# facebookresearch/goliath

Hardware: AMD Instinct MI355X
Metric: relit views/sec (fwd+bwd) at 2048x1334, 250k Gaussians (higher is better)
Workload: dtype f32; 1 GPU; rgca_config2_envrelight; gaussians=250000, views_per_gpu=8, micro_batches=2, world_size=1, dist_backend=none, rccl_world_size=0, parallelism=view-parallel x1, launch=hip_graph_replay

## Files before the change

goliath_amd/_lib.py:

```python
import ctypes
import os

import torch

_HERE = os.path.dirname(os.path.abspath(__file__))
LIB_PATH = os.environ.get("GOLIATH_HIP_LIB") or os.path.join(_HERE, "lib", "libgoliath_hip.so")

_lib = None

_SYMBOLS = [
    "gol_version", "gol_last_error", "gol_sg_eval_fwd", "gol_sg_eval_bwd", "gol_project_fwd",
    "gol_project_bwd", "gol_project_bwd_records", "gol_bin_sort", "gol_splat_pack", "gol_render_layout", "gol_render_fwd", "gol_render_bwd", "gol_rasterize_fwd", "gol_rasterize_bwd", "gol_rasterize_nd_fwd", "gol_rasterize_nd_bwd", "gol_raster_plan", "gol_raster_count_pairs", "gol_shade_fwd",
    "gol_shade_bwd", "gol_shade_project_fwd", "gol_shade_project_bwd", "gol_render_layout_projected", "gol_render_fwd_projected",
    "gol_render_bwd_projected", "gol_selftest_wave_sum4", "gol_selftest_wave_sum8", "gol_raydirs_fwd", "gol_mvp_aabb", "gol_mvp_march_fwd",
    "gol_mvp_march_bwd", "gol_mvp_march_warp_fwd", "gol_mvp_march_warp_bwd", "gol_envmap_pack", "gol_uvlight_phong_fwd", "gol_uvlight_phong_bwd",
    "gol_uvlight_ggx_fwd", "gol_uvlight_ggx_bwd", "gol_l1_blocks", "gol_l1_fwd", "gol_l1_bwd",
    "gol_tail_conv_fwd", "gol_tail_conv_bwd", "gol_tail_conv_bwd_scratch_floats", "gol_ssim_blocks", "gol_ssim_fwd", "gol_ssim_bwd",
    "gol_shadow_pcf", "gol_imgtail_partial_floats", "gol_imgtail_fwd", "gol_imgtail_bwd", "gol_mvp_shadow_march", "gol_mesh_raster_workspace_bytes", "gol_mesh_raster",
    "gol_mesh_render_fwd", "gol_mesh_render_bwd", "gol_mesh_render_edge_bwd",
    "gol_vert_normals_fwd", "gol_vert_normals_bwd", "gol_values_to_uv_fwd", "gol_values_to_uv_bwd", "gol_uvgeom_fwd",
    "gol_uvgeom_bwd", "gol_lbs_skeleton_fwd", "gol_lbs_skeleton_bwd", "gol_lbs_skin_fwd", "gol_lbs_skin_bwd",
    "gol_optim_chunk_elems", "gol_optim_grad_stats", "gol_optim_finalize", "gol_optim_adam_step",
    "gol_regloss_chunk_elems", "gol_regloss_fwd", "gol_regloss_bwd", "gol_backlit_fwd", "gol_backlit_bwd",
    "gol_imgloss_chunk_elems", "gol_imgloss_fwd", "gol_imgloss_finalize", "gol_imgloss_bwd", "gol_depth_disc_mask",
    "gol_mask_erode", "gol_envbg_blur_taps", "gol_envbg_scratch_floats", "gol_envbg_image", "gol_envbg_compose",
    "gol_sh_norm_constants", "gol_sh_basis_fwd", "gol_light_sh_fwd", "gol_envspin_scratch_floats", "gol_envspin_frame",
    "gol_mvp_template_fwd", "gol_mvp_template_bwd", "gol_mvp_primtransf_fwd", "gol_mvp_primtransf_bwd",
    "gol_envprefilter_scratch_floats", "gol_envprefilter_sg",
    "gol_trunk_conv_fwd", "gol_trunk_conv_bwd_scratch_floats", "gol_trunk_conv_bwd",
    "gol_enc_conv_fwd", "gol_enc_conv_bwd_scratch_floats", "gol_enc_conv_bwd",
    "gol_mesh_raster_flat", "gol_uv_face_index_workspace_bytes", "gol_uv_face_index", "gol_uv_topology", "gol_nearest_valid", "gol_impaint_gather",
    "gol_face_visibility", "gol_view_texture", "gol_texmean_finalize",
    "gol_uvframes_bwd_scratch_floats", "gol_uvframes_fwd", "gol_uvframes_bwd",
    "gol_upconv_fwd", "gol_upconv_bwd_scratch_floats", "gol_upconv_bwd",
    "gol_upcat_conv_fwd", "gol_upcat_conv_bwd_scratch_floats", "gol_upcat_conv_bwd",
    "gol_uvtex_partial_floats", "gol_uvtex_fwd", "gol_uvtex_bwd", "gol_pack_rgba_fwd", "gol_pack_rgba_bwd",
    "gol_normal_rgba",
    "gol_olat_features_fwd", "gol_olat_combine_fwd", "gol_olat_combine_bwd",
    "gol_mvp_tail_fwd", "gol_mvp_tail_bwd_scratch_floats", "gol_mvp_tail_bwd",
    "gol_conv3_fwd", "gol_conv3_bwd_x",
    "gol_mbconv_front_tiles", "gol_mbconv_front_fwd", "gol_mbconv_front_bwd_x",
]


class GoliathHipError(RuntimeError):
    pass


def load():
    global _lib
    if _lib is None:
        if not os.path.exists(LIB_PATH):
            raise GoliathHipError(
                f"{LIB_PATH} not found: the HIP extension is not built. Run "
                "`python -m goliath_amd.build` (or __graft_entry__.build()). There is no CPU fallback."
            )
        lib = ctypes.CDLL(LIB_PATH)
        lib.gol_version.restype = ctypes.c_char_p
        lib.gol_last_error.restype = ctypes.c_char_p
        for name in _SYMBOLS:
            getattr(lib, name)
        _lib = lib
    return _lib


def exported_symbols():
    return list(_SYMBOLS)
# ... 72 lines not shown
```

goliath_amd/csrc/abi.hip:

```cpp
#include <cstdarg>
#include <cstdio>

#include "gol_common.h"

static thread_local char g_err[512] = "";

void gol_set_error(const char* fmt, ...) {
  va_list ap;
  va_start(ap, fmt);
  vsnprintf(g_err, sizeof(g_err), fmt, ap);
  va_end(ap);
}

extern "C" const char* gol_version(void) { return "goliath_hip 0.1.0 gfx950"; }
extern "C" const char* gol_last_error(void) { return g_err; }

__global__ void selftest_wave_sum4_kernel(const float* __restrict__ in, float* __restrict__ out) {
  const int l = threadIdx.x;
  const float r = gol_wave_sum4(in[l], in[64 + l], in[128 + l], in[192 + l]);
  out[l] = r;
  out[64 + l] = gol_wave_sum_to_lane63(in[l]);
}
extern "C" int gol_selftest_wave_sum4(const float* in256, float* out128, void* stream) {
  selftest_wave_sum4_kernel<<<1, 64, 0, (hipStream_t)stream>>>(in256, out128);
  GOL_CHECK_LAUNCH();
  return GOL_OK;
}

__global__ void selftest_wave_sum8_kernel(const float* __restrict__ in, float* __restrict__ out) {
  const int l = threadIdx.x;
  out[l] = gol_wave_sum8(in[l], in[64 + l], in[128 + l], in[192 + l], in[256 + l], in[320 + l], in[384 + l], in[448 + l]);
}
extern "C" int gol_selftest_wave_sum8(const float* in512, float* out64, void* stream) {
  selftest_wave_sum8_kernel<<<1, 64, 0, (hipStream_t)stream>>>(in512, out64);
  GOL_CHECK_LAUNCH();
  return GOL_OK;
}
```

goliath_amd/csrc/gol_common.h:

```cpp
#pragma once
#include <hip/hip_runtime.h>
#include <type_traits>
#include <stdint.h>

#include "../../include/goliath_hip.h"

#define GOL_BLUR 0.3f
#define GOL_FOV_CLAMP 1.3f
#define GOL_EIG_FLOOR 0.1f
#define GOL_RADIUS_SIGMAS 3.0f
#define GOL_Z_EPS 1e-6f
#define GOL_ALPHA_CAP_FWD 0.999f
#define GOL_ALPHA_CAP_BWD 0.99f
#define GOL_ALPHA_FLOOR (1.f / 255.f)
#define GOL_T_STOP 1e-4f
#define GOL_COMP_EPS 1e-6f

#define GOL_WAVE 64

void gol_set_error(const char* fmt, ...);

#define GOL_REQUIRE(cond, msg)                                         \
  do {                                                                 \
    if (!(cond)) {                                                     \
// ... 23 lines not shown
__device__ __forceinline__ float gol_add_row_shr8(float v) {
  float r;
  asm("s_nop 1\n\tv_add_f32_dpp %0, %1, %1 row_shr:8 row_mask:0xf bank_mask:0xf bound_ctrl:1" : "=v"(r) : "v"(v));
  return r;
}
__device__ __forceinline__ float gol_add_row_bcast15(float v) {
  asm("s_nop 1\n\tv_add_f32_dpp %0, %0, %0 row_bcast:15 row_mask:0xa bank_mask:0xf" : "+v"(v));
  return v;
}
__device__ __forceinline__ float gol_add_row_bcast31(float v) {
  asm("s_nop 1\n\tv_add_f32_dpp %0, %0, %0 row_bcast:31 row_mask:0xc bank_mask:0xf" : "+v"(v));
  return v;
}

__device__ __forceinline__ float gol_row_sum_to_lane15(float v) {
  v += gol_dpp_mov0<0x111>(v);
  v += gol_dpp_mov0<0x112>(v);
  v += gol_dpp_mov0<0x114>(v);
  return gol_add_row_shr8(v);
}

__device__ __forceinline__ float gol_swap32_sum(float x, float y) {
  const auto r = __builtin_amdgcn_permlane32_swap(__builtin_bit_cast(unsigned, x), __builtin_bit_cast(unsigned, y),
                                                  false, false);
  const unsigned r0 = r[0], r1 = r[1];
  return __uint_as_float(r0) + __uint_as_float(r1);
}
__device__ __forceinline__ float gol_swap16_sum(float x, float y) {
  const auto r = __builtin_amdgcn_permlane16_swap(__builtin_bit_cast(unsigned, x), __builtin_bit_cast(unsigned, y),
                                                  false, false);
  const unsigned r0 = r[0], r1 = r[1];
  return __uint_as_float(r0) + __uint_as_float(r1);
}
__device__ __forceinline__ float gol_wave_sum4(float a, float b, float c, float d) {
  const float ac = gol_swap32_sum(a, c);
  const float bd = gol_swap32_sum(b, d);
  const float q = gol_swap16_sum(ac, bd);
  return gol_row_sum_to_lane15(q);
}

__device__ __forceinline__ float gol_wave_sum8(float a0, float a1, float a2, float a3, float a4, float a5, float a6,
                                               float a7) {
  const float p02 = gol_swap32_sum(a0, a2), p13 = gol_swap32_sum(a1, a3);
  const float q02 = gol_swap32_sum(a4, a6), q13 = gol_swap32_sum(a5, a7);
  float p = gol_swap16_sum(p02, p13);
  const float q = gol_swap16_sum(q02, q13);
  p += gol_dpp_mov0<0x128>(p);
  asm("s_nop 1\n\tv_add_f32_dpp %0, %1, %1 row_ror:8 row_mask:0xf bank_mask:0xc" : "+v"(p) : "v"(q));
  p += gol_dpp_mov0<0x111>(p);
  p += gol_dpp_mov0<0x112>(p);
  float r;
  asm("s_nop 1\n\tv_add_f32_dpp %0, %1, %1 row_shr:4 row_mask:0xf bank_mask:0xf bound_ctrl:1" : "=v"(r) : "v"(p));
  return r;
}

template <typename T>
__device__ __forceinline__ T* gol_at(T* base, unsigned byte_off) {
  return reinterpret_cast<T*>(reinterpret_cast<char*>(const_cast<typename std::remove_const<T>::type*>(base)) + byte_off);
}

template <typename T>
__device__ __forceinline__ T* gol_uniform(T* q) {
  const uint64_t v = reinterpret_cast<uint64_t>(q);
  const uint32_t lo = __builtin_amdgcn_readfirstlane((uint32_t)v), hi = __builtin_amdgcn_readfirstlane((uint32_t)(v >> 32));
  return reinterpret_cast<T*>(((uint64_t)hi << 32) | lo);
}

__device__ __forceinline__ unsigned long long gol_ballot(bool p) { return __builtin_amdgcn_ballot_w64(p); }

__device__ __forceinline__ float gol_wave_sum_to_lane63(float v) {
  v += gol_dpp_mov0<0x111>(v);
  v += gol_dpp_mov0<0x112>(v);
  v += gol_dpp_mov0<0x114>(v);
  v = gol_add_row_shr8(v);
  v = gol_add_row_bcast15(v);
  return gol_add_row_bcast31(v);
}

template <int CTRL, int ROW_MASK>
__device__ __forceinline__ double gol_dpp_add0(double v) {
  const int lo = __builtin_amdgcn_update_dpp(0, __double2loint(v), CTRL, ROW_MASK, 0xf, false);
  const int hi = __builtin_amdgcn_update_dpp(0, __double2hiint(v), CTRL, ROW_MASK, 0xf, false);
  return v + __hiloint2double(hi, lo);
}
__device__ __forceinline__ double gol_wave_sum_to_lane63(double v) {
  v = gol_dpp_add0<0x111, 0xf>(v);
  v = gol_dpp_add0<0x112, 0xf>(v);
  v = gol_dpp_add0<0x114, 0xf>(v);
  v = gol_dpp_add0<0x118, 0xf>(v);
  v = gol_dpp_add0<0x142, 0xa>(v);
  return gol_dpp_add0<0x143, 0xc>(v);
}

__device__ __forceinline__ float gol_readlane63(float v) {
  return __builtin_bit_cast(float, __builtin_amdgcn_readlane(__builtin_bit_cast(int, v), 63));
}

__device__ __forceinline__ float gol_alpha_tau(float op) {
  _Pragma("clang fp contract(on)")
  const float k = 255.f * op;
  return (k >= 1.f) ? __logf(k) * 1.001f + 1e-3f : -1.f;
}
__device__ __forceinline__ float gol_min_sigma_rect(float gx, float gy, float a, float b, float c, float ia, float ic,
                                                    float x0, float x1, float y0, float y1) {
  if (gx >= x0 && gx <= x1 && gy >= y0 && gy <= y1) return 0.f;
  float m = 3.0e38f;
// ... 38 lines not shown
```

goliath_amd/csrc/gol_raster.h:

```cpp
#pragma once
#include <type_traits>

#include "gol_common.h"

namespace {

constexpr int kBatch = 256;
constexpr float kUnA = GOL_UN_A, kUnB = GOL_UN_B;
__device__ __forceinline__ float3 true_conic(float a, float b, float c) { return make_float3(a * kUnA, b * kUnB, c * kUnA); }
#ifdef GOL_EXACT_MATH
__device__ __forceinline__ float exact_sigma(float a, float b, float c, float dx, float dy) {
#pragma clang fp contract(off)
  const float t1 = (a * dx) * dx, t2 = (c * dy) * dy, t3 = (b * dx) * dy;
  const float h = 0.5f * (t1 + t2);
  return h + t3;
}
__device__ __forceinline__ float exact_exp_neg(float s) { return (float)exp(-(double)s); }
__device__ __forceinline__ float exact_next_T(float T, float alpha) {
#pragma clang fp contract(off)
  const float om = 1.f - alpha;
  return T * om;
}
#endif

// ... 94 lines not shown
template <int PPL> using ivec = typename Pix<PPL>::iv;

template <int PPL>
__device__ __forceinline__ void visit_falloff(float ca, float cb, float cc, float dx, const fvec<PPL>& dy, fvec<PPL>& sigma,
                                              fvec<PPL>& e) {
#ifndef GOL_EXACT_MATH
  sigma = (ca * dx * dx + cc * dy * dy) + (cb * dx) * dy;
#pragma unroll
  for (int q = 0; q < PPL; ++q) e[q] = __builtin_amdgcn_exp2f(-sigma[q]);
#else
#pragma unroll
  for (int q = 0; q < PPL; ++q) { sigma[q] = exact_sigma(ca, cb, cc, dx, dy[q]); e[q] = exact_exp_neg(sigma[q]); }
#endif
}

template <int PPL>
__device__ __forceinline__ unsigned long long fwd_step(const fvec<PPL>& sigma, fvec<PPL> alpha, const fvec<PPL>& live,
                                                       const fvec<PPL>& T_cur, fvec<PPL>& vis, fvec<PPL>& next_T,
                                                       bool (&take)[PPL], unsigned long long (&stop)[PPL]) {
  alpha *= live;
  vis = alpha * T_cur;
#ifndef GOL_EXACT_MATH
  next_T = T_cur - vis;
#else
#pragma unroll
  for (int q = 0; q < PPL; ++q) next_T[q] = exact_next_T(T_cur[q], alpha[q]);
#endif
  unsigned long long any_stop = 0ull;
#pragma unroll
  for (int q = 0; q < PPL; ++q) {
    const unsigned long long mc = gol_ballot(!(sigma[q] < 0.f)) & gol_ballot(!(alpha[q] < GOL_ALPHA_FLOOR));
    const unsigned long long ms = gol_ballot(next_T[q] <= GOL_T_STOP);
    take[q] = __builtin_amdgcn_inverse_ballot_w64(mc & ~ms);
    stop[q] = mc & ms;
    any_stop |= stop[q];
  }
  return any_stop;
}

template <int PPL>
__device__ __forceinline__ void fwd_take(const bool (&take)[PPL], const fvec<PPL>& next_T, fvec<PPL>& vis, fvec<PPL>& T_cur) {
#pragma unroll
  for (int q = 0; q < PPL; ++q) vis[q] = take[q] ? vis[q] : 0.f;
#ifndef GOL_EXACT_MATH
  T_cur -= vis;
#else
#pragma unroll
  for (int q = 0; q < PPL; ++q) T_cur[q] = take[q] ? next_T[q] : T_cur[q];
#endif
}

template <int PPL>
__device__ __forceinline__ unsigned long long bwd_taken(float opacity, const fvec<PPL>& e, const fvec<PPL>& sigma, int li,
                                                        const ivec<PPL>& bin_final, fvec<PPL>& alpha,
                                                        unsigned long long (&mv)[PPL]) {
  alpha = opacity * e;
  unsigned long long many = 0ull;
#pragma unroll
  for (int q = 0; q < PPL; ++q) {
    alpha[q] = fminf(GOL_ALPHA_CAP_BWD, alpha[q]);
    mv[q] = gol_ballot(li <= bin_final[q]) & gol_ballot(!(sigma[q] < 0.f)) & gol_ballot(!(alpha[q] < GOL_ALPHA_FLOOR));
    many |= mv[q];
  }
  return many;
}

template <int PPL>
__device__ __forceinline__ void bwd_recur(const unsigned long long (&mv)[PPL], fvec<PPL>& alpha, fvec<PPL>& T_cur,
                                          bool (&v)[PPL], fvec<PPL>& ra, fvec<PPL>& fac) {
#pragma unroll
  for (int q = 0; q < PPL; ++q) {
    v[q] = __builtin_amdgcn_inverse_ballot_w64(mv[q]);
    alpha[q] = v[q] ? alpha[q] : 0.f;
  }
  const fvec<PPL> one_m = 1.f - alpha;
#pragma unroll
  for (int q = 0; q < PPL; ++q) ra[q] = __builtin_amdgcn_rcpf(one_m[q]);
  const fvec<PPL> T_new = T_cur * ra;
  fac = alpha * T_new;
  T_cur = T_new;
}

template <int PPL>
__device__ __forceinline__ void bwd_moments(const fvec<PPL>& e, const fvec<PPL>& w, const fvec<PPL>& T_cur,
                                            const fvec<PPL>& alpha, const bool (&v)[PPL], const fvec<PPL>& dy,
                                            fvec<PPL>& R, fvec<PPL>& gop, fvec<PPL>& gy, fvec<PPL>& gyy) {
  const fvec<PPL> d = w - R;
  const fvec<PPL> v_alpha = T_cur * d;
  R += alpha * d;
  gop = e * v_alpha;
#pragma unroll
  for (int q = 0; q < PPL; ++q) gop[q] = v[q] ? gop[q] : 0.f;
  gy = gop * dy;
  gyy = gy * dy;
}
template <int PPL>
__device__ __forceinline__ float lane_sum(const fvec<PPL>& x) {
  float s = x[0];
#pragma unroll
  for (int q = 1; q < PPL; ++q) s += x[q];
  return s;
}

template <int PPL>
__device__ __forceinline__ int wave_last_entry(const ivec<PPL>& bin_final) {
  int wmax = bin_final[0];
#pragma unroll
  for (int q = 1; q < PPL; ++q) wmax = max(wmax, bin_final[q]);
#pragma unroll
  for (int off = 32; off > 0; off >>= 1) wmax = max(wmax, __shfl_xor(wmax, off, 64));
  return __builtin_amdgcn_readfirstlane(wmax);
}

inline int64_t raster_grid(int B, int img_h, int img_w) {
  return (int64_t)B * 8 * (((img_h + 15) / 16 + 7) / 8) * ((img_w + 15) / 16);
}

#define GOL_RASTER_CHECK_DIMS(bytes_per_pixel, too_large_msg)                                                           \
  do {                                                                                                                  \
    GOL_REQUIRE(B >= 0 && N >= 0, "negative size");                                                                     \
    GOL_REQUIRE(block == 16, "only block_width == 16 is implemented (the reference's value, render_gsplat.py:28)");     \
    GOL_REQUIRE(img_h > 0 && img_w > 0, "empty image");                                                                 \
    GOL_REQUIRE(raster_grid(B, img_h, img_w) < (1ll << 31), "too many tiles");                                          \
    GOL_REQUIRE((uint64_t)img_h * (uint64_t)img_w * (uint64_t)(bytes_per_pixel) < (1ull << 32), too_large_msg);         \
  } while (0)

template <typename F>
inline void with_ppl(int ppl, F&& fn) {
  if (ppl == 2) fn(std::integral_constant<int, 2>());
  else fn(std::integral_constant<int, 1>());
}
constexpr std::true_type kYes{}; constexpr std::false_type kNo{};

}
```

goliath_amd/csrc/raster.hip:

```cpp
#include <cstdlib>

#include "gol_raster.h"

namespace {

constexpr int kBgGroup = 4;

template <bool EXTRA, bool LAZY, int PPL>
__global__ __launch_bounds__(64 * Pix<PPL>::kWaves) void raster_fwd_kernel(
    int N, int img_h, int img_w, int planar, int tiles_x, int tiles_y, const int2* __restrict__ tile_bins,
    const int32_t* __restrict__ sorted_ids, int64_t capacity, const float* __restrict__ records,
    const float* __restrict__ background, float* __restrict__ out_img,
    float* __restrict__ out_extra, float* __restrict__ final_Ts, int32_t* __restrict__ final_idx,
    float* __restrict__ out_alpha, float* __restrict__ out_extra_norm, float norm_lo,
    const float* __restrict__ l1_target, const float* __restrict__ l1_mask, int l1_mask_c,
    uint8_t* __restrict__ l1_sign, float* __restrict__ l1_partial, int n_views, int bg_group, int bg_vec16,
    uint8_t* __restrict__ stage_mask) {
  typedef typename Pix<PPL>::fv fv;
  typedef typename Pix<PPL>::iv iv;
  constexpr int NW = Pix<PPL>::kWaves, NT = 64 * NW;
  __shared__ float s_l1[NW];
  __shared__ float4 s_a[kBatch];
  __shared__ float4 s_b[kBatch];
  __shared__ float2 s_c[kBatch];
// ... 325 lines not shown
  const size_t goff = (size_t)view * N;
  bool in[PPL];
  size_t pp[PPL];
  fv py, T_final;
  iv bin_final;
#pragma unroll
  for (int q = 0; q < PPL; ++q) {
    in[q] = (i0 + q < img_h) && (j < img_w);
    py[q] = (float)(i0 + q) + 0.5f;
    pp[q] = in[q] ? ((size_t)view * img_h + i0 + q) * img_w + j : 0;
    T_final[q] = in[q] ? final_Ts[pp[q]] : 1.f;
    bin_final[q] = in[q] ? final_idx[pp[q]] : (range.x - 1);
  }
  fv T_cur = T_final;
  fv vo0 = 0.f, vo1 = 0.f, vo2 = 0.f, vo3 = 0.f, voa = 0.f;
  {
    const float vsc = (v_img_scale ? v_img_scale[0] : 1.f) * v_img_scale_mul;
    const size_t os = planar ? hw : 1;
#pragma unroll
    for (int q = 0; q < PPL; ++q) {
      if (!in[q]) continue;
      const size_t p = pp[q];
      const int i = i0 + q;
      const size_t o = planar ? (size_t)view * 3 * hw + (size_t)i * img_w + j : 3 * p;
      float g0 = 0.f, g1 = 0.f, g2 = 0.f;
      if (v_out_img) { g0 = v_out_img[o]; g1 = v_out_img[o + os]; g2 = v_out_img[o + 2 * os]; }
      if (v_sign) {
        const unsigned code = v_sign[p];
        float m0 = vsc, m1 = vsc, m2 = vsc;
        if (v_sign_mask) {
          const float* mk = v_sign_mask + (size_t)view * v_sign_mask_c * hw + (size_t)i * img_w + j;
          m0 *= mk[0]; m1 *= (v_sign_mask_c == 3) ? mk[hw] : mk[0]; m2 *= (v_sign_mask_c == 3) ? mk[2 * hw] : mk[0];
        }
        g0 += (float)((int)(code & 3u) - 1) * m0;
        g1 += (float)((int)((code >> 2) & 3u) - 1) * m1;
        g2 += (float)((int)((code >> 4) & 3u) - 1) * m2;
      }
      vo0[q] = g0; vo1[q] = g1; vo2[q] = g2;
      if (EXTRA && v_out_extra) vo3[q] = v_out_extra[p];
      if (v_out_alpha) voa[q] = v_out_alpha[p];
    }
  }
  fv R = (background[0] * vo0 + background[1] * vo1 + background[2] * vo2) - voa;

  const int wmax = wave_last_entry<PPL>(bin_final);
  if (lane == 0) s_wmax[wave] = wmax;
  __syncthreads();
  int bmax = s_wmax[0];
#pragma unroll
  for (int w = 1; w < NW; ++w) bmax = max(bmax, s_wmax[w]);
  bmax = min(bmax, range.y - 1);
  if (bmax < range.x) return;

  float* acc_lane = &s_acc[wave][0][lane >> 3];
  const int n_batches = (bmax - range.x + kBatchB) / kBatchB;
  auto entry_id = [&](int bb2) {
    const int e = bmax - bb2 * kBatchB - tid;
    return (tid < kBatchB && e >= range.x) ? ids[e] : 0;
  };
  const uint8_t* __restrict__ i_mask = stage_mask ? stage_mask + (size_t)view * capacity : nullptr;
  auto entry_mask = [&](int bb2) {
    const int e = bmax - bb2 * kBatchB - tid;
    return (i_mask && tid < kBatchB && e >= range.x) ? (int)i_mask[e] : 0;
  };
  int gid_next = entry_id(0), mask_next = entry_mask(0);
  unsigned rec_bytes = GOL_GRAD_RECORD * sizeof(float);
  if (PACKED) asm volatile("" : "+s"(rec_bytes));
  for (int bb = 0; bb < n_batches; ++bb) {
    __syncthreads();
    const int batch_end = bmax - bb * kBatchB;
    const int batch_size = min(kBatchB, batch_end + 1 - range.x);
    const int gid = gid_next, mask = mask_next;
    if (tid < kBatchB) {
      if (tid < batch_size) {
        const Staged st = i_mask ? stage_entry_masked(records, goff + (size_t)gid, mask)
                                 : stage_entry<PPL>(records, goff + (size_t)gid, (float)(tc.tx * 16), (float)(tc.ty * 16));
        s_e[tid].a = st.a; s_e[tid].b = st.b; s_e[tid].c = st.c; s_mask[tid] = st.mask;
        s_id[tid] = gid;
      } else {
        s_mask[tid] = 0;
      }
    }
    if (bb + 1 < n_batches) { gid_next = entry_id(bb + 1); mask_next = entry_mask(bb + 1); }
    __syncthreads();

    const int t0 = max(0, batch_end - wmax);
    unsigned long long bits = gol_ballot((s_mask[lane] >> wave) & 1);
    if (t0 > 0) bits &= ~0ull << t0;
    unsigned long long touched = 0ull;
    while (bits) {
      const int t = __builtin_ctzll(bits);
      bits &= bits - 1;
      const float4 a4 = s_e[t].a;
      const float4 b4 = s_e[t].b;
      const float2 c2 = s_e[t].c;
      const int li = batch_end - t;
      const float dx = a4.x - px;
      const fv dy = a4.y - py;
      fv sigma, vis, alpha, ra, fac;
      visit_falloff<PPL>(a4.z, a4.w, b4.x, dx, dy, sigma, vis);
      unsigned long long mv[PPL];
      if (bwd_taken<PPL>(b4.y, vis, sigma, li, bin_final, alpha, mv) == 0ull) continue;
      bool v[PPL];
      bwd_recur<PPL>(mv, alpha, T_cur, v, ra, fac);
      fv w = b4.z * vo0 + b4.w * vo1 + c2.x * vo2;
      if (EXTRA) w += c2.y * vo3;
      fv gop, gy, gyy;
      bwd_moments<PPL>(vis, w, T_cur, alpha, v, dy, R, gop, gy, gyy);
      float g0s, g1s, g2s, g3 = 0.f;
      if (PPL == 2) {
        g0s = __builtin_fmaf(fac[0], vo0[0], fac[PPL - 1] * vo0[PPL - 1]);
        g1s = __builtin_fmaf(fac[0], vo1[0], fac[PPL - 1] * vo1[PPL - 1]);
        g2s = __builtin_fmaf(fac[0], vo2[0], fac[PPL - 1] * vo2[PPL - 1]);
        if (EXTRA) g3 = __builtin_fmaf(fac[0], vo3[0], fac[PPL - 1] * vo3[PPL - 1]);
      } else {
        g0s = fac[0] * vo0[0]; g1s = fac[0] * vo1[0]; g2s = fac[0] * vo2[0];
        if (EXTRA) g3 = fac[0] * vo3[0];
      }
      const float m0 = lane_sum<PPL>(gop), my = lane_sum<PPL>(gy), myy = lane_sum<PPL>(gyy);
      const float mx = m0 * dx, mxx = mx * dx, mxy = my * dx;
      const float r0 = gol_wave_sum8(g0s, g2s, mx, mxx, g1s, m0, my, mxy);
      const float r2 = gol_wave_sum_to_lane63(myy);
      const float r3 = EXTRA ? gol_wave_sum_to_lane63(g3) : 0.f;
      if ((lane & 7) == 7) {
        float* a = gol_at(acc_lane, (unsigned)t * (unsigned)(kAcc * sizeof(float)));
        a[0] = r0;
        if (lane == 63) { a[8 - 7] = r2; a[9 - 7] = r3; }
      }
      touched |= 1ull << t;
    }
    s_touched[wave][lane] = (int32_t)((touched >> lane) & 1ull);
    __syncthreads();
    if (PACKED) {
      if (tid < kBatchB) {
        int tw[NW];
#pragma unroll
        for (int w = 0; w < NW; ++w) tw[w] = s_touched[w][tid];
        float s[kAcc];
#pragma unroll
        for (int k = 0; k < kAcc; ++k) s[k] = 0.f;
        bool any = false;
#pragma unroll
        for (int w = 0; w < NW; ++w) {
          if (tw[w]) {
            any = true;
            const float4* q = reinterpret_cast<const float4*>(&s_acc[w][tid][0]);
            const float4 q0 = q[0], q1 = q[1], q2 = q[2];
            s[0] += q0.x; s[1] += q0.y; s[2] += q0.z; s[3] += q0.w;
            s[4] += q1.x; s[5] += q1.y; s[6] += q1.z; s[7] += q1.w;
            s[8] += q2.x; s[9] += q2.y;
          }
        }
        if (any) {
          const float4 a4 = s_e[tid].a;
          const float4 b4 = s_e[tid].b;
          const float nop = -b4.y, cc = b4.x;
          const float wxx = nop * a4.z * kUnA, wxy = nop * a4.w * kUnB, wyy = nop * cc * kUnA, hnop = 0.5f * nop;
          float4* o = reinterpret_cast<float4*>(&s_acc[0][tid][0]);
          o[0] = make_float4(s[0], s[1], s[2], s[3]);
          o[1] = make_float4(wxx * s[4] + wxy * s[5], wxy * s[4] + wyy * s[5], hnop * s[6], nop * s[7]);
          *reinterpret_cast<float2*>(o + 2) = make_float2(hnop * s[8], s[9]);
          s_touched[0][tid] = 1;
        }
      }
      __syncthreads();
      const int c = tid & 15;
      if (c <= (EXTRA ? 9 : 8)) {
        float* rec_c = v_colors + goff * 16 + c;
        constexpr int kIt = kBatchB * 16 / NT, kCh = 4;
        static_assert(kIt % kCh == 0, "the merge issues its atomics in chunks of kCh entries per lane");
#pragma unroll
        for (int i0 = 0; i0 < kIt; i0 += kCh) {
          int flag[kCh], id[kCh];
          float val[kCh];
#pragma unroll
          for (int i = 0; i < kCh; ++i) {
            const int t = (tid >> 4) + (i0 + i) * (NT / 16);
            flag[i] = s_touched[0][t]; id[i] = s_id[t]; val[i] = s_acc[0][t][c];
          }
#pragma unroll
          for (int i = 0; i < kCh; ++i) {
            if (flag[i]) {
              char* r = reinterpret_cast<char*>(rec_c) + (uint64_t)(unsigned)id[i] * rec_bytes;
              atomicAdd(reinterpret_cast<float*>(r), val[i]);
            }
          }
        }
      }
    } else if (tid < batch_size) {
      float a[kAcc];
#pragma unroll
      for (int k = 0; k < kAcc; ++k) a[k] = 0.f;
      bool any = false;
#pragma unroll
      for (int w = 0; w < NW; ++w) {
        if (s_touched[w][tid]) {
          any = true;
          const float4* q = reinterpret_cast<const float4*>(&s_acc[w][tid][0]);
          const float4 q0 = q[0], q1 = q[1], q2 = q[2];
          a[0] += q0.x; a[1] += q0.y; a[2] += q0.z; a[3] += q0.w;
          a[4] += q1.x; a[5] += q1.y; a[6] += q1.z; a[7] += q1.w;
          a[8] += q2.x; a[9] += q2.y;
        }
      }
      if (any) {
        const size_t g = goff + (size_t)s_id[tid];
        const float4 a4 = s_e[tid].a;
        const float4 b4 = s_e[tid].b;
        const float nop = -b4.y;
        const float3 cn = true_conic(a4.z, a4.w, b4.x);
        atomicAdd(v_colors + 3 * g, a[0]); atomicAdd(v_colors + 3 * g + 1, a[1]); atomicAdd(v_colors + 3 * g + 2, a[2]);
        atomicAdd(v_opacity + g, a[3]);
        atomicAdd(v_xy + 2 * g, nop * (cn.x * a[4] + cn.y * a[5]));
        atomicAdd(v_xy + 2 * g + 1, nop * (cn.y * a[4] + cn.z * a[5]));
        atomicAdd(v_conic + 3 * g, 0.5f * nop * a[6]); atomicAdd(v_conic + 3 * g + 1, nop * a[7]);
        atomicAdd(v_conic + 3 * g + 2, 0.5f * nop * a[8]);
        if (EXTRA && v_extra) atomicAdd(v_extra + g, a[9]);
      }
    }
  }
}

__global__ __launch_bounds__(256) void raster_count_pairs_kernel(int N, int img_h, int img_w, int tiles_x, int tiles_y,
                                                                 const int2* __restrict__ tile_bins,
                                                                 const int32_t* __restrict__ sorted_ids, int64_t capacity,
                                                                 const float* __restrict__ records,
                                                                 const int32_t* __restrict__ final_idx,
                                                                 unsigned long long* __restrict__ counts) {
  __shared__ unsigned long long s_cnt[2];
  const int view = blockIdx.y, tile = blockIdx.x, T = tiles_x * tiles_y;
  const int ty = tile / tiles_x, tx = tile - ty * tiles_x;
  const int j = tx * 16 + (threadIdx.x & 15), i = ty * 16 + (threadIdx.x >> 4);
  if (threadIdx.x < 2) s_cnt[threadIdx.x] = 0ull;
  __syncthreads();
  const int2 range = tile_bins[(size_t)view * T + tile];
  unsigned long long tested = 0, taken = 0;
  if (i < img_h && j < img_w && range.y > range.x) {
    const int last = min(range.y - 1, final_idx[((size_t)view * img_h + i) * img_w + j]);
    const float px = (float)j + 0.5f, py = (float)i + 0.5f;
    for (int li = range.x; li <= last; ++li) {
      const float4* R = reinterpret_cast<const float4*>(records + ((size_t)view * N + sorted_ids[(size_t)view * capacity + li]) * GOL_SPLAT_RECORD);
      const float4 q0 = R[0], q1 = R[1];
      const float dx = q0.x - px, dy = q0.y - py;
      f1 sg, e;
      visit_falloff<1>(q0.z, q0.w, q1.x, dx, f1(dy), sg, e);
      const float alpha = fminf(GOL_ALPHA_CAP_FWD, q1.y * e[0]);
      ++tested;
      taken += (!(sg[0] < 0.f) && !(alpha < GOL_ALPHA_FLOOR)) ? 1 : 0;
    }
  }
  atomicAdd(&s_cnt[0], tested);
  atomicAdd(&s_cnt[1], taken);
  __syncthreads();
  if (threadIdx.x < 2 && s_cnt[threadIdx.x]) atomicAdd(counts + 2 * view + threadIdx.x, s_cnt[threadIdx.x]);
}

__global__ __launch_bounds__(256) void splat_pack_kernel(size_t n, const float* __restrict__ xys,
                                                         const float* __restrict__ conics,
                                                         const float* __restrict__ colors,
                                                         const float* __restrict__ extra,
                                                         const float* __restrict__ opacities,
                                                         float* __restrict__ records) {
  const size_t e = (size_t)blockIdx.x * 256 + threadIdx.x;
  if (e >= n) return;
  gol_record_write(records + e * GOL_SPLAT_RECORD, xys[2 * e], xys[2 * e + 1], conics[3 * e], conics[3 * e + 1],
                   conics[3 * e + 2], opacities[e], colors ? colors[3 * e] : 0.f, colors ? colors[3 * e + 1] : 0.f,
                   colors ? colors[3 * e + 2] : 0.f, extra ? extra[e] : 0.f);
}

// ... 151 lines not shown
```

goliath_amd/csrc/raster_nd.hip:

```cpp
#include "gol_raster.h"

namespace {

constexpr int kChunkMax = 16;
constexpr int kBatchNdB = 64;

template <int CK>
__device__ __forceinline__ void stage_colors(float* __restrict__ row, const float* __restrict__ colors, size_t g, int C,
                                             int c0, int nc) {
  const float* col = colors + g * (size_t)C + c0;
#pragma unroll
  for (int c = 0; c < CK; ++c) row[c] = (c < nc) ? col[c] : 0.f;
}

template <int CK, int PPL>
__global__ __launch_bounds__(64 * Pix<PPL>::kWaves) void raster_nd_fwd_kernel(
    int N, int C, int c_first, int img_h, int img_w, int tiles_x, int tiles_y, const int2* __restrict__ tile_bins,
    const int32_t* __restrict__ sorted_ids, int64_t capacity, const float* __restrict__ records,
    const float* __restrict__ colors, const float* __restrict__ background, float* __restrict__ out_img,
    float* __restrict__ final_Ts, int32_t* __restrict__ final_idx, int n_views) {
  typedef typename Pix<PPL>::fv fv;
  typedef typename Pix<PPL>::iv iv;
  constexpr int NW = Pix<PPL>::kWaves, NT = 64 * NW;
  __shared__ float4 s_a[kBatch];
// ... 150 lines not shown
      for (int c = 0; c < CK; ++c) vo[c][q] = (c < nc) ? g[c] : 0.f;
      if (v_out_alpha && c0 == 0) voa[q] = v_out_alpha[p];
    }
  }

  const int wmax = wave_last_entry<PPL>(bin_final);
  if (lane == 0) s_wmax[wave] = wmax;
  __syncthreads();
  int bmax = s_wmax[0];
#pragma unroll
  for (int w = 1; w < NW; ++w) bmax = max(bmax, s_wmax[w]);
  bmax = min(bmax, range.y - 1);
  if (bmax < range.x) return;

  fv bgdot = 0.f;
#pragma unroll
  for (int c = 0; c < CK; ++c) bgdot += ((c < nc) ? background[c0 + c] : 0.f) * vo[c];
  fv T_cur = T_final;
  fv R = bgdot - voa;

  constexpr bool kSum8 = NG % 2 == 0;
  float* acc_lane = &s_acc[wave][0][kSum8 ? lane >> 3 : lane >> 4];
  const int n_batches = (bmax - range.x + kBatchNdB) / kBatchNdB;
  for (int bb = 0; bb < n_batches; ++bb) {
    __syncthreads();
    const int batch_end = bmax - bb * kBatchNdB;
    const int batch_size = min(kBatchNdB, batch_end + 1 - range.x);
    if (tid < kBatchNdB) {
      if (tid < batch_size) {
        const int gid = ids[batch_end - tid];
        const size_t g = goff + (size_t)gid;
        const Staged st = stage_entry<PPL>(records, g, (float)(tc.tx * 16), (float)(tc.ty * 16));
        s_a[tid] = st.a; s_b[tid] = make_float2(st.b.x, st.b.y); s_mask[tid] = st.mask;
        s_id[tid] = gid;
        stage_colors<CK>(s_col + tid * CK, colors, g, C, c0, nc);
      } else {
        s_mask[tid] = 0;
      }
    }
    (&s_touched[0][0])[tid] = 0;
    __syncthreads();

    const int t0 = max(0, batch_end - wmax);
    unsigned long long bits = gol_ballot((s_mask[lane] >> wave) & 1);
    if (t0 > 0) bits &= ~0ull << t0;
    while (bits) {
      const int t = __builtin_ctzll(bits);
      bits &= bits - 1;
      const float4 a4 = s_a[t];
      const float2 b2 = s_b[t];
      const int li = batch_end - t;
      const float dx = a4.x - px;
      const fv dy = a4.y - py;
      fv sigma, vis, alpha, ra, fac;
      visit_falloff<PPL>(a4.z, a4.w, b2.x, dx, dy, sigma, vis);
      unsigned long long mv[PPL];
      if (bwd_taken<PPL>(b2.y, vis, sigma, li, bin_final, alpha, mv) == 0ull) continue;
      bool v[PPL];
      bwd_recur<PPL>(mv, alpha, T_cur, v, ra, fac);
      const float* col = s_col + t * CK;
      fv w = 0.f;
#pragma unroll
      for (int c = 0; c < CK; ++c) w += col[c] * vo[c];
      fv gop, gy, gyy;
      bwd_moments<PPL>(vis, w, T_cur, alpha, v, dy, R, gop, gy, gyy);
      float s[kRow];
#pragma unroll
      for (int c = 0; c < CK; ++c) {
        s[c] = fac[0] * vo[c][0];
#pragma unroll
        for (int q = 1; q < PPL; ++q) s[c] = __builtin_fmaf(fac[q], vo[c][q], s[c]);
      }
      const float m0 = lane_sum<PPL>(gop), my = lane_sum<PPL>(gy), myy = lane_sum<PPL>(gyy);
      const float mx = m0 * dx;
      s[CK + 0] = m0; s[CK + 1] = mx; s[CK + 2] = my; s[CK + 3] = mx * dx; s[CK + 4] = my * dx; s[CK + 5] = myy;
#pragma unroll
      for (int k = NS; k < kRow; ++k) s[k] = 0.f;
      if constexpr (kSum8) {
        float r[NG / 2];
#pragma unroll
        for (int p = 0; p < NG / 2; ++p)
          r[p] = gol_wave_sum8(s[8 * p], s[8 * p + 2], s[8 * p + 4], s[8 * p + 6],
                               s[8 * p + 1], s[8 * p + 3], s[8 * p + 5], s[8 * p + 7]);
        if ((lane & 7) == 7) {
          float* a = gol_at(acc_lane, (unsigned)t * (unsigned)(kRow * sizeof(float)));
#pragma unroll
          for (int p = 0; p < NG / 2; ++p) a[8 * p] = r[p];
          s_touched[wave][t] = 1;
        }
      } else {
        float r[NG];
#pragma unroll
        for (int gi = 0; gi < NG; ++gi) r[gi] = gol_wave_sum4(s[4 * gi], s[4 * gi + 1], s[4 * gi + 2], s[4 * gi + 3]);
        if ((lane & 15) == 15) {
          float* a = gol_at(acc_lane, (unsigned)t * (unsigned)(kRow * sizeof(float)));
#pragma unroll
          for (int gi = 0; gi < NG; ++gi) a[4 * gi] = r[gi];
          s_touched[wave][t] = 1;
        }
      }
    }
    __syncthreads();
    for (int idx = tid; idx < batch_size * NS; idx += NT) {
      const int t = idx / NS, k = idx - t * NS;
      if (k < CK && k >= nc) continue;
      bool any = false;
#pragma unroll
      for (int w = 0; w < NW; ++w) any = any || (s_touched[w][t] != 0);
      if (!any) continue;
      const size_t g = goff + (size_t)s_id[t];
      const float4 a4 = s_a[t];
      const float2 b2 = s_b[t];
      const float nop = -b2.y;
      const float3 cn = true_conic(a4.z, a4.w, b2.x);
      const float ca = cn.x, cb = cn.y, cc = cn.z;
      int k1 = k, k2 = k;
      float w1 = 1.f, w2 = 0.f;
      float* dst;
      if (k < CK) {
        dst = v_colors + g * (size_t)C + c0 + k;
      } else {
        const int m = k - CK;
        k1 = (m == 1 || m == 2) ? CK + 1 : k;
        k2 = CK + 2;
        w1 = (m == 0) ? 1.f : (m == 1) ? nop * ca : (m == 2) ? nop * cb : (m == 4) ? nop : 0.5f * nop;
        w2 = (m == 1) ? nop * cb : (m == 2) ? nop * cc : 0.f;
        dst = (m == 0) ? v_opacity + g : (m <= 2) ? v_xy + 2 * g + (m - 1) : v_conic + 3 * g + (m - 3);
      }
      float s1 = 0.f, s2 = 0.f;
#pragma unroll
      for (int w = 0; w < NW; ++w) {
        const bool tw = s_touched[w][t] != 0;
        s1 += tw ? s_acc[w][t][k1] : 0.f;
        s2 += tw ? s_acc[w][t][k2] : 0.f;
      }
      atomicAdd(dst, w1 * s1 + w2 * s2);
    }
  }
}

struct NdPlan { int n16, tail, tail_first; };
NdPlan nd_plan(int C) {
  const int r = C % kChunkMax;
  NdPlan p;
  p.n16 = C / kChunkMax + (r > 8 ? 1 : 0);
  p.tail = (r == 0 || r > 8) ? 0 : r <= 1 ? 1 : r <= 2 ? 2 : r <= 4 ? 4 : 8;
  p.tail_first = (C / kChunkMax) * kChunkMax;
  return p;
}

template <typename F>
bool for_nd_launches(int C, F&& fn) {
  const NdPlan pl = nd_plan(C);
  if (pl.n16 > 0) fn(std::integral_constant<int, 16>(), pl.n16, 0);
  switch (pl.tail) {
    case 0: break;
    case 1: fn(std::integral_constant<int, 1>(), 1, pl.tail_first); break;
    case 2: fn(std::integral_constant<int, 2>(), 1, pl.tail_first); break;
    case 4: fn(std::integral_constant<int, 4>(), 1, pl.tail_first); break;
    case 8: fn(std::integral_constant<int, 8>(), 1, pl.tail_first); break;
    default: return false;
  }
  return true;
}

}

extern "C" int gol_rasterize_nd_fwd(int B, int N, int C, int img_h, int img_w, int block, const int32_t* tile_bins,
                                    const int32_t* sorted_ids, int64_t capacity, const float* records, const float* colors,
                                    const float* background, float* out_img, float* final_Ts, int32_t* final_idx,
                                    int pixels_per_lane, void* stream) {
  GOL_REQUIRE(C >= 1, "C >= 1 colour channels");
  GOL_REQUIRE(C <= 16 * 65535, "too many colour channels (at most 1048560: one launch row of 16-channel chunks)");
  GOL_RASTER_CHECK_DIMS((uint64_t)C * 4ull, "image too large (32-bit byte offsets inside a view: H * W * C * 4 bytes)");
  if (B == 0) return GOL_OK;
  GOL_REQUIRE(tile_bins && background && out_img && final_Ts && final_idx, "null pointer");
  GOL_REQUIRE(capacity == 0 || sorted_ids, "null sorted_ids");
  GOL_REQUIRE(N == 0 || (records && colors), "null Gaussian records / colors");
  GOL_REQUIRE(pixels_per_lane >= 0 && pixels_per_lane <= 2, "pixels_per_lane: 0 (choose by B), 1 or 2");
  int ppl = pixels_per_lane;
  if (ppl == 0) gol_raster_plan(B, &ppl);
  const int tiles_x = (img_w + 15) / 16, tiles_y = (img_h + 15) / 16;
  const unsigned gx = (unsigned)raster_grid(B, img_h, img_w);
  const int2* bins = reinterpret_cast<const int2*>(tile_bins);
  hipStream_t s = (hipStream_t)stream;
  const bool covered = for_nd_launches(C, [&](auto ck_c, int n_chunks, int c_first) {
    with_ppl(ppl, [&](auto ppl_c) {
      constexpr int CK = decltype(ck_c)::value, PPL = decltype(ppl_c)::value;
      raster_nd_fwd_kernel<CK, PPL><<<dim3(gx, n_chunks), 64 * Pix<PPL>::kWaves, 0, s>>>(
// ... 37 lines not shown
```

include/goliath_hip.h:

```cpp
#ifndef GOLIATH_HIP_H
#define GOLIATH_HIP_H

#include <stddef.h>
#include <stdint.h>

#ifdef __cplusplus
extern "C" {
#endif

typedef enum {
  GOL_OK = 0,
  GOL_ERR_INVALID_ARG = -1,
  GOL_ERR_LAUNCH = -2,
  GOL_ERR_UNSUPPORTED = -3
} gol_status;

const char* gol_version(void);
const char* gol_last_error(void);
int gol_selftest_wave_sum4(const float* in256, float* out128, void* stream);
int gol_selftest_wave_sum8(const float* in512, float* out64, void* stream);

int gol_sg_eval_fwd(int N, int D, int L, const float* lobe_dirs, const float* lobe_sigmas,
                    const float* light_values, const float* light_pts, const float* prim_pts,
                    const int32_t* n_lights, float* integral, int w_type, void* stream);
int gol_sg_eval_bwd(int N, int D, int L, const float* lobe_dirs, const float* lobe_sigmas,
                    const float* light_values, const float* light_pts, const float* prim_pts,
                    const int32_t* n_lights, const float* grad_integral, float* grad_dirs,
                    float* grad_sigmas, float* grad_light_values, int w_type, void* stream);

int gol_project_fwd(int B, int N, const float* means3d, const float* scales, float glob_scale,
                    const float* quats, const float* viewmats, const float* intrins, int img_h,
                    int img_w, int block, float clip_thresh, float* cov3d, float* xys,
                    float* depths, int32_t* radii, float* conics, float* compensation,
                    int32_t* num_tiles_hit, const float* opacities, float* opac_eff, const float* colors,
                    float* records, void* stream);
int gol_project_bwd(int B, int N, const float* means3d, const float* scales, float glob_scale,
                    const float* quats, const float* viewmats, const float* intrins,
                    const float* cov3d, const int32_t* radii, const float* conics,
                    const float* compensation, const float* v_xy, const float* v_depth,
                    const float* v_conic, const float* v_compensation, const float* opacities,
                    const float* v_opac_eff, int grad_stride, float* v_mean3d, float* v_scale, float* v_quat,
                    float* v_opacity, void* stream);
int gol_project_bwd_records(int B, int N, const float* means3d, const float* scales, float glob_scale,
                            const float* quats, const float* viewmats, const float* intrins, const int32_t* radii,
                            const float* conics, const float* compensation, const float* opacities,
                            const float* grad_records, int with_depth, float* v_mean3d, float* v_scale, float* v_quat,
                            float* v_opacity, float* v_colors, void* stream);

int gol_bin_sort(int B, int N, const float* xys, const float* depths, const int32_t* radii,
                 const float* conics, const float* opacities, int img_h, int img_w, int block,
                 int64_t capacity, int32_t* tile_count, int32_t* tile_bins, uint64_t* isect_keys,
                 int32_t* sorted_ids, int32_t* n_isect, uint64_t* reach_scratch, void* stream);

#define GOL_GRAD_RECORD 16
#define GOL_SPLAT_RECORD 16
int gol_splat_pack(int B, int N, const float* xys, const float* conics, const float* colors, const float* extra,
                   const float* opacities, float* records, void* stream);
int gol_rasterize_fwd(int B, int N, int img_h, int img_w, int block, int planar, const int32_t* tile_bins,
                      const int32_t* sorted_ids, int64_t capacity, const float* records, int with_extra,
                      const float* background, float* out_img,
                      float* out_extra, float* final_Ts, int32_t* final_idx, float* out_alpha,
                      float* out_extra_norm, float norm_lo, const float* l1_target, const float* l1_mask, int l1_mask_c,
                      uint8_t* l1_sign, float* l1_partial, float* l1_out, float l1_scale, uint8_t* stage_mask,
                      int pixels_per_lane, void* stream);
int gol_rasterize_bwd(int B, int N, int img_h, int img_w, int block, int planar, const int32_t* tile_bins,
                      const int32_t* sorted_ids, int64_t capacity, const float* records, int with_extra,
                      const float* background, const float* final_Ts,
                      const int32_t* final_idx, const float* v_out_img, const float* v_out_extra,
                      const float* v_out_alpha, float* v_xy, float* v_conic, float* v_colors,
                      float* v_extra, float* v_opacity, int grad_stride, const uint8_t* v_sign, const float* v_sign_mask,
                      int v_sign_mask_c, const float* v_img_scale, float v_img_scale_mul, const uint8_t* stage_mask,
                      int stage_mask_ppl, int pixels_per_lane, void* stream);
int gol_raster_count_pairs(int B, int N, int img_h, int img_w, const int32_t* tile_bins, const int32_t* sorted_ids,
// ... 455 lines not shown
```

Before: 3155 views/s.

## Fold opacity factor out of raster backward inner loop and fuse wave column reduction

The rasterizer backward inner loop now carries the uncapped raw alpha (opacity*falloff) as the gradient weight, so the per-lane validity select and the opacity multiply drop out. The -opacity scale is applied once per Gaussian at the flush stage, with the opacity gradient divided by opacity. For PPL==2, a new hand-written DPP sequence (gol_wave_colsum) folds the dx-weighted moments and myy into one cross-lane reduction that writes to remapped accumulator columns, replacing wave_sum8 plus an extra lane-63 reduction. This cuts ALU and DPP work per splat-pixel step, but relies on intricate inline asm and on a division by opacity that can lose precision when opacity is tiny.

```diff
diff --git a/goliath_amd/_lib.py b/goliath_amd/_lib.py
--- a/goliath_amd/_lib.py
+++ b/goliath_amd/_lib.py
@@ -12,7 +12,7 @@
     "gol_version", "gol_last_error", "gol_sg_eval_fwd", "gol_sg_eval_bwd", "gol_project_fwd",
     "gol_project_bwd", "gol_project_bwd_records", "gol_bin_sort", "gol_splat_pack", "gol_render_layout", "gol_render_fwd", "gol_render_bwd", "gol_rasterize_fwd", "gol_rasterize_bwd", "gol_rasterize_nd_fwd", "gol_rasterize_nd_bwd", "gol_raster_plan", "gol_raster_count_pairs", "gol_shade_fwd",
     "gol_shade_bwd", "gol_shade_project_fwd", "gol_shade_project_bwd", "gol_render_layout_projected", "gol_render_fwd_projected",
-    "gol_render_bwd_projected", "gol_selftest_wave_sum4", "gol_selftest_wave_sum8", "gol_raydirs_fwd", "gol_mvp_aabb", "gol_mvp_march_fwd",
+    "gol_render_bwd_projected", "gol_selftest_wave_sum4", "gol_selftest_wave_sum8", "gol_selftest_wave_colsum", "gol_raydirs_fwd", "gol_mvp_aabb", "gol_mvp_march_fwd",
     "gol_mvp_march_bwd", "gol_mvp_march_warp_fwd", "gol_mvp_march_warp_bwd", "gol_envmap_pack", "gol_uvlight_phong_fwd", "gol_uvlight_phong_bwd",
     "gol_uvlight_ggx_fwd", "gol_uvlight_ggx_bwd", "gol_l1_blocks", "gol_l1_fwd", "gol_l1_bwd",
     "gol_tail_conv_fwd", "gol_tail_conv_bwd", "gol_tail_conv_bwd_scratch_floats", "gol_ssim_blocks", "gol_ssim_fwd", "gol_ssim_bwd",
diff --git a/goliath_amd/csrc/abi.hip b/goliath_amd/csrc/abi.hip
--- a/goliath_amd/csrc/abi.hip
+++ b/goliath_amd/csrc/abi.hip
@@ -36,3 +36,14 @@
   GOL_CHECK_LAUNCH();
   return GOL_OK;
 }
+
+__global__ void selftest_wave_colsum_kernel(const float* __restrict__ in, const float* __restrict__ dx,
+                                            float* __restrict__ out) {
+  const int l = threadIdx.x;
+  out[l] = gol_wave_colsum(in[l], in[64 + l], in[128 + l], in[192 + l], in[256 + l], in[320 + l], dx[l]);
+}
+extern "C" int gol_selftest_wave_colsum(const float* in384, const float* dx64, float* out64, void* stream) {
+  selftest_wave_colsum_kernel<<<1, 64, 0, (hipStream_t)stream>>>(in384, dx64, out64);
+  GOL_CHECK_LAUNCH();
+  return GOL_OK;
+}
diff --git a/goliath_amd/csrc/gol_common.h b/goliath_amd/csrc/gol_common.h
--- a/goliath_amd/csrc/gol_common.h
+++ b/goliath_amd/csrc/gol_common.h
@@ -99,6 +99,31 @@
   float r;
   asm("s_nop 1\n\tv_add_f32_dpp %0, %1, %1 row_shr:4 row_mask:0xf bank_mask:0xf bound_ctrl:1" : "=v"(r) : "v"(p));
   return r;
+}
+
+__device__ __forceinline__ float gol_wave_colsum(float s0, float s1, float s2, float m0, float my, float myy, float dx) {
+  const float a01 = gol_swap32_sum(s0, s1), a2y = gol_swap32_sum(s2, myy);
+  const float c = gol_swap32_sum(m0, my);
+  float p = gol_swap16_sum(a01, a2y);
+  float q = gol_swap16_sum(c, c);
+  float u;
+  asm("s_nop 1\n\t"
+      "v_mul_f32_dpp %1, %1, %3 quad_perm:[0,1,2,3] row_mask:0xa bank_mask:0xf\n\t"
+      "v_add_f32_dpp %0, %0, %0 row_ror:8 row_mask:0xf bank_mask:0xf\n\t"
+      "v_mul_f32_e32 %2, %1, %3\n\t"
+      "v_add_f32_dpp %0, %1, %1 row_ror:8 row_mask:0xf bank_mask:0xc\n\t"
+      "s_nop 0\n\t"
+      "v_add_f32_dpp %2, %2, %2 row_ror:8 row_mask:0xf bank_mask:0xf\n\t"
+      "v_add_f32_dpp %0, %0, %0 row_ror:4 row_mask:0xf bank_mask:0xa\n\t"
+      "s_nop 0\n\t"
+      "v_add_f32_dpp %0, %2, %2 row_ror:4 row_mask:0xf bank_mask:0x1\n\t"
+      "s_nop 1\n\t"
+      "v_add_f32_dpp %0, %0, %0 row_shr:1 row_mask:0xf bank_mask:0xf bound_ctrl:1\n\t"
+      "s_nop 1\n\t"
+      "v_add_f32_dpp %0, %0, %0 row_shr:2 row_mask:0xf bank_mask:0xf bound_ctrl:1"
+      : "+v"(p), "+v"(q), "=&v"(u)
+      : "v"(dx));
+  return p;
 }
 
 template <typename T>
diff --git a/goliath_amd/csrc/gol_raster.h b/goliath_amd/csrc/gol_raster.h
--- a/goliath_amd/csrc/gol_raster.h
+++ b/goliath_amd/csrc/gol_raster.h
@@ -170,26 +170,26 @@
 
 template <int PPL>
 __device__ __forceinline__ unsigned long long bwd_taken(float opacity, const fvec<PPL>& e, const fvec<PPL>& sigma, int li,
-                                                        const ivec<PPL>& bin_final, fvec<PPL>& alpha,
+                                                        const ivec<PPL>& bin_final, fvec<PPL>& raw,
                                                         unsigned long long (&mv)[PPL]) {
-  alpha = opacity * e;
+  static_assert(GOL_ALPHA_CAP_BWD > GOL_ALPHA_FLOOR, "bwd_taken tests the uncapped alpha against the floor");
+  raw = opacity * e;
   unsigned long long many = 0ull;
 #pragma unroll
   for (int q = 0; q < PPL; ++q) {
-    alpha[q] = fminf(GOL_ALPHA_CAP_BWD, alpha[q]);
-    mv[q] = gol_ballot(li <= bin_final[q]) & gol_ballot(!(sigma[q] < 0.f)) & gol_ballot(!(alpha[q] < GOL_ALPHA_FLOOR));
+    mv[q] = gol_ballot(li <= bin_final[q]) & gol_ballot(!(sigma[q] < 0.f)) & gol_ballot(!(raw[q] < GOL_ALPHA_FLOOR));
     many |= mv[q];
   }
   return many;
 }
 
 template <int PPL>
-__device__ __forceinline__ void bwd_recur(const unsigned long long (&mv)[PPL], fvec<PPL>& alpha, fvec<PPL>& T_cur,
-                                          bool (&v)[PPL], fvec<PPL>& ra, fvec<PPL>& fac) {
+__device__ __forceinline__ void bwd_recur(const unsigned long long (&mv)[PPL], fvec<PPL>& raw, fvec<PPL>& T_cur,
+                                          fvec<PPL>& alpha, fvec<PPL>& ra, fvec<PPL>& fac) {
 #pragma unroll
   for (int q = 0; q < PPL; ++q) {
-    v[q] = __builtin_amdgcn_inverse_ballot_w64(mv[q]);
-    alpha[q] = v[q] ? alpha[q] : 0.f;
+    raw[q] = __builtin_amdgcn_inverse_ballot_w64(mv[q]) ? raw[q] : 0.f;
+    asm("v_min_f32_e32 %0, %2, %1" : "=v"(alpha[q]) : "v"(raw[q]), "i"(__builtin_bit_cast(int, GOL_ALPHA_CAP_BWD)));
   }
   const fvec<PPL> one_m = 1.f - alpha;
 #pragma unroll
@@ -200,15 +200,13 @@
 }
 
 template <int PPL>
-__device__ __forceinline__ void bwd_moments(const fvec<PPL>& e, const fvec<PPL>& w, const fvec<PPL>& T_cur,
-                                            const fvec<PPL>& alpha, const bool (&v)[PPL], const fvec<PPL>& dy,
+__device__ __forceinline__ void bwd_moments(const fvec<PPL>& raw_m, const fvec<PPL>& w, const fvec<PPL>& T_cur,
+                                            const fvec<PPL>& alpha, const fvec<PPL>& dy,
                                             fvec<PPL>& R, fvec<PPL>& gop, fvec<PPL>& gy, fvec<PPL>& gyy) {
   const fvec<PPL> d = w - R;
   const fvec<PPL> v_alpha = T_cur * d;
   R += alpha * d;
-  gop = e * v_alpha;
-#pragma unroll
-  for (int q = 0; q < PPL; ++q) gop[q] = v[q] ? gop[q] : 0.f;
+  gop = raw_m * v_alpha;
   gy = gop * dy;
   gyy = gy * dy;
 }
diff --git a/goliath_amd/csrc/raster.hip b/goliath_amd/csrc/raster.hip
--- a/goliath_amd/csrc/raster.hip
+++ b/goliath_amd/csrc/raster.hip
@@ -401,7 +401,10 @@
   bmax = min(bmax, range.y - 1);
   if (bmax < range.x) return;
 
-  float* acc_lane = &s_acc[wave][0][lane >> 3];
+  constexpr unsigned kColSlot = 0x78514230u;
+  const bool res_lane = (lane & 7) == 7 || (PPL == 2 && lane == 19);
+  const int acc_col = PPL == 1 ? lane >> 3 : lane == 19 ? 6 : (int)((kColSlot >> (4 * (lane >> 3))) & 15u);
+  float* acc_lane = &s_acc[wave][0][acc_col];
   const int n_batches = (bmax - range.x + kBatchB) / kBatchB;
   auto entry_id = [&](int bb2) {
     const int e = bmax - bb2 * kBatchB - tid;
@@ -446,16 +449,15 @@
       const int li = batch_end - t;
       const float dx = a4.x - px;
       const fv dy = a4.y - py;
-      fv sigma, vis, alpha, ra, fac;
+      fv sigma, vis, raw, alpha, ra, fac;
       visit_falloff<PPL>(a4.z, a4.w, b4.x, dx, dy, sigma, vis);
       unsigned long long mv[PPL];
-      if (bwd_taken<PPL>(b4.y, vis, sigma, li, bin_final, alpha, mv) == 0ull) continue;
-      bool v[PPL];
-      bwd_recur<PPL>(mv, alpha, T_cur, v, ra, fac);
+      if (bwd_taken<PPL>(b4.y, vis, sigma, li, bin_final, raw, mv) == 0ull) continue;
+      bwd_recur<PPL>(mv, raw, T_cur, alpha, ra, fac);
       fv w = b4.z * vo0 + b4.w * vo1 + c2.x * vo2;
       if (EXTRA) w += c2.y * vo3;
       fv gop, gy, gyy;
-      bwd_moments<PPL>(vis, w, T_cur, alpha, v, dy, R, gop, gy, gyy);
+      bwd_moments<PPL>(raw, w, T_cur, alpha, dy, R, gop, gy, gyy);
       float g0s, g1s, g2s, g3 = 0.f;
       if (PPL == 2) {
         g0s = __builtin_fmaf(fac[0], vo0[0], fac[PPL - 1] * vo0[PPL - 1]);
@@ -467,14 +469,26 @@
         if (EXTRA) g3 = fac[0] * vo3[0];
       }
       const float m0 = lane_sum<PPL>(gop), my = lane_sum<PPL>(gy), myy = lane_sum<PPL>(gyy);
-      const float mx = m0 * dx, mxx = mx * dx, mxy = my * dx;
-      const float r0 = gol_wave_sum8(g0s, g2s, mx, mxx, g1s, m0, my, mxy);
-      const float r2 = gol_wave_sum_to_lane63(myy);
-      const float r3 = EXTRA ? gol_wave_sum_to_lane63(g3) : 0.f;
-      if ((lane & 7) == 7) {
-        float* a = gol_at(acc_lane, (unsigned)t * (unsigned)(kAcc * sizeof(float)));
-        a[0] = r0;
-        if (lane == 63) { a[8 - 7] = r2; a[9 - 7] = r3; }
+      if constexpr (PPL == 2) {
+        const float r3 = EXTRA ? gol_wave_sum_to_lane63(g3) : 0.f;
+        const float r0 = gol_wave_colsum(g0s, g1s, g2s, m0, my, myy, dx);
+        if (res_lane) {
+          unsigned row_t = (unsigned)t * (unsigned)(kAcc * sizeof(float));
+          asm("" : "+s"(row_t));
+          float* a = gol_at(acc_lane, row_t);
+          a[0] = r0;
+          if (EXTRA && lane == 63) a[9 - 7] = r3;
+        }
+      } else {
+        const float mx = m0 * dx, mxx = mx * dx, mxy = my * dx;
+        const float r0 = gol_wave_sum8(g0s, g2s, mx, mxx, g1s, m0, my, mxy);
+        const float r2 = gol_wave_sum_to_lane63(myy);
+        const float r3 = EXTRA ? gol_wave_sum_to_lane63(g3) : 0.f;
+        if (res_lane) {
+          float* a = gol_at(acc_lane, (unsigned)t * (unsigned)(kAcc * sizeof(float)));
+          a[0] = r0;
+          if (lane == 63) { a[8 - 7] = r2; a[9 - 7] = r3; }
+        }
       }
       touched |= 1ull << t;
     }
@@ -503,12 +517,12 @@
         if (any) {
           const float4 a4 = s_e[tid].a;
           const float4 b4 = s_e[tid].b;
-          const float nop = -b4.y, cc = b4.x;
-          const float wxx = nop * a4.z * kUnA, wxy = nop * a4.w * kUnB, wyy = nop * cc * kUnA, hnop = 0.5f * nop;
+          const float cc = b4.x;
+          const float wxx = -a4.z * kUnA, wxy = -a4.w * kUnB, wyy = -cc * kUnA;
           float4* o = reinterpret_cast<float4*>(&s_acc[0][tid][0]);
-          o[0] = make_float4(s[0], s[1], s[2], s[3]);
-          o[1] = make_float4(wxx * s[4] + wxy * s[5], wxy * s[4] + wyy * s[5], hnop * s[6], nop * s[7]);
-          *reinterpret_cast<float2*>(o + 2) = make_float2(hnop * s[8], s[9]);
+          o[0] = make_float4(s[0], s[1], s[2], s[3] / b4.y);
+          o[1] = make_float4(wxx * s[4] + wxy * s[5], wxy * s[4] + wyy * s[5], -0.5f * s[6], -s[7]);
+          *reinterpret_cast<float2*>(o + 2) = make_float2(-0.5f * s[8], s[9]);
           s_touched[0][tid] = 1;
         }
       }
@@ -556,14 +570,13 @@
         const size_t g = goff + (size_t)s_id[tid];
         const float4 a4 = s_e[tid].a;
         const float4 b4 = s_e[tid].b;
-        const float nop = -b4.y;
         const float3 cn = true_conic(a4.z, a4.w, b4.x);
         atomicAdd(v_colors + 3 * g, a[0]); atomicAdd(v_colors + 3 * g + 1, a[1]); atomicAdd(v_colors + 3 * g + 2, a[2]);
-        atomicAdd(v_opacity + g, a[3]);
-        atomicAdd(v_xy + 2 * g, nop * (cn.x * a[4] + cn.y * a[5]));
-        atomicAdd(v_xy + 2 * g + 1, nop * (cn.y * a[4] + cn.z * a[5]));
-        atomicAdd(v_conic + 3 * g, 0.5f * nop * a[6]); atomicAdd(v_conic + 3 * g + 1, nop * a[7]);
-        atomicAdd(v_conic + 3 * g + 2, 0.5f * nop * a[8]);
+        atomicAdd(v_opacity + g, a[3] / b4.y);
+        atomicAdd(v_xy + 2 * g, -(cn.x * a[4] + cn.y * a[5]));
+        atomicAdd(v_xy + 2 * g + 1, -(cn.y * a[4] + cn.z * a[5]));
+        atomicAdd(v_conic + 3 * g, -0.5f * a[6]); atomicAdd(v_conic + 3 * g + 1, -a[7]);
+        atomicAdd(v_conic + 3 * g + 2, -0.5f * a[8]);
         if (EXTRA && v_extra) atomicAdd(v_extra + g, a[9]);
       }
     }
diff --git a/goliath_amd/csrc/raster_nd.hip b/goliath_amd/csrc/raster_nd.hip
--- a/goliath_amd/csrc/raster_nd.hip
+++ b/goliath_amd/csrc/raster_nd.hip
@@ -226,18 +226,17 @@
       const int li = batch_end - t;
       const float dx = a4.x - px;
       const fv dy = a4.y - py;
-      fv sigma, vis, alpha, ra, fac;
+      fv sigma, vis, raw, alpha, ra, fac;
       visit_falloff<PPL>(a4.z, a4.w, b2.x, dx, dy, sigma, vis);
       unsigned long long mv[PPL];
-      if (bwd_taken<PPL>(b2.y, vis, sigma, li, bin_final, alpha, mv) == 0ull) continue;
-      bool v[PPL];
-      bwd_recur<PPL>(mv, alpha, T_cur, v, ra, fac);
+      if (bwd_taken<PPL>(b2.y, vis, sigma, li, bin_final, raw, mv) == 0ull) continue;
+      bwd_recur<PPL>(mv, raw, T_cur, alpha, ra, fac);
       const float* col = s_col + t * CK;
       fv w = 0.f;
 #pragma unroll
       for (int c = 0; c < CK; ++c) w += col[c] * vo[c];
       fv gop, gy, gyy;
-      bwd_moments<PPL>(vis, w, T_cur, alpha, v, dy, R, gop, gy, gyy);
+      bwd_moments<PPL>(raw, w, T_cur, alpha, dy, R, gop, gy, gyy);
       float s[kRow];
 #pragma unroll
       for (int c = 0; c < CK; ++c) {
@@ -285,7 +284,6 @@
       const size_t g = goff + (size_t)s_id[t];
       const float4 a4 = s_a[t];
       const float2 b2 = s_b[t];
-      const float nop = -b2.y;
       const float3 cn = true_conic(a4.z, a4.w, b2.x);
       const float ca = cn.x, cb = cn.y, cc = cn.z;
       int k1 = k, k2 = k;
@@ -297,8 +295,8 @@
         const int m = k - CK;
         k1 = (m == 1 || m == 2) ? CK + 1 : k;
         k2 = CK + 2;
-        w1 = (m == 0) ? 1.f : (m == 1) ? nop * ca : (m == 2) ? nop * cb : (m == 4) ? nop : 0.5f * nop;
-        w2 = (m == 1) ? nop * cb : (m == 2) ? nop * cc : 0.f;
+        w1 = (m == 0) ? 1.f : (m == 1) ? -ca : (m == 2) ? -cb : (m == 4) ? -1.f : -0.5f;
+        w2 = (m == 1) ? -cb : (m == 2) ? -cc : 0.f;
         dst = (m == 0) ? v_opacity + g : (m <= 2) ? v_xy + 2 * g + (m - 1) : v_conic + 3 * g + (m - 3);
       }
       float s1 = 0.f, s2 = 0.f;
@@ -308,7 +306,7 @@
         s1 += tw ? s_acc[w][t][k1] : 0.f;
         s2 += tw ? s_acc[w][t][k2] : 0.f;
       }
-      atomicAdd(dst, w1 * s1 + w2 * s2);
+      atomicAdd(dst, k == CK ? s1 / b2.y : w1 * s1 + w2 * s2);
     }
   }
 }
diff --git a/include/goliath_hip.h b/include/goliath_hip.h
--- a/include/goliath_hip.h
+++ b/include/goliath_hip.h
@@ -19,6 +19,7 @@
 const char* gol_last_error(void);
 int gol_selftest_wave_sum4(const float* in256, float* out128, void* stream);
 int gol_selftest_wave_sum8(const float* in512, float* out64, void* stream);
+int gol_selftest_wave_colsum(const float* in384, const float* dx64, float* out64, void* stream);
 
 int gol_sg_eval_fwd(int N, int D, int L, const float* lobe_dirs, const float* lobe_sigmas,
                     const float* light_values, const float* light_pts, const float* prim_pts,
```

Measured after the change: 3285 views/s, median of 6. 4.1% higher.
